# chonlei/neural-ode-ion-channels

Measured on AMD Instinct MI355X. Metric: trajectories/sec (sinewave protocol, 100k steps), higher is better.
Workload: dtype f64

## Files before the change

### include/ionode.h

```cpp
#ifndef IONODE_H
#define IONODE_H

#include <stddef.h>
#include <stdint.h>

#ifdef __cplusplus
extern "C" {
#endif

#define IONODE_ABI_VERSION 10

#define IONODE_MODEL_HH2 0
#define IONODE_MODEL_MARKOV6 1
#define IONODE_MODEL_NNF 2
#define IONODE_MODEL_NND 3

#define IONODE_STATUS_OK 0
#define IONODE_STATUS_DT_UNDERFLOW 1
#define IONODE_STATUS_NONFINITE 2
#define IONODE_STATUS_MAX_STEPS 3

#define IONODE_OK 0
#define IONODE_ERR_ARG (-1)
#define IONODE_ERR_UNSUPPORTED (-2)
// ... 27 lines not shown
  double *ckpt;
  int32_t ckpt_cap;
  int32_t t_eval_exact;
  const double *sse_ref;
  double *sse_out;
  double max_step;
  const double *v_at_outputs;
  int64_t mlp_image_stride;
  int32_t traj_per_image;
  const int32_t *launch_order;
} ionode_desc;

#define IONODE_DEFAULT_MAX_TOTAL_STEPS 1000000

size_t ionode_mlp_packed_floats(int32_t mlp_layers, int32_t mlp_width);

int ionode_mlp_pack(const float *state_dict_flat, int32_t mlp_layers, int32_t mlp_width, float *packed);

int ionode_dopri5(const ionode_desc *d, const float *mlp_packed, const double *params, const double *prot_v,
                  const double *prot_t, const int32_t *prot_of_traj, const void *y0, const double *t_eval,
                  void *y_out, double *i_out, int32_t *status, int64_t *stats, void *stream);

int ionode_dense_defer_plan(const ionode_desc *d, int32_t want_current, int64_t out[2]);
int ionode_dopri5_deferred(const ionode_desc *d, const float *mlp_packed, const double *params, const double *prot_v,
                           const double *prot_t, const int32_t *prot_of_traj, const void *y0, const double *t_eval,
                           void *y_out, double *i_out, int32_t *status, int64_t *stats, void *stream, void *workspace,
                           int64_t workspace_bytes);

int ionode_protocol_at_outputs(const ionode_desc *d, const double *prot_v, const double *prot_t, const double *t_eval,
                               double *v_out, void *stream);

int ionode_launch_geometry(const ionode_desc *d, int32_t out[4]);

const char *ionode_kernel_name(const ionode_desc *d);

const char *ionode_last_kernel_name(void);

int32_t ionode_lane_wise_from(int32_t model, int32_t mlp_width);

const char *ionode_last_error(void);
int32_t ionode_abi_version(void);


size_t ionode_grad_image_floats(int32_t mlp_layers, int32_t mlp_width);
int ionode_grad_pack(const float *state_dict_flat, int32_t mlp_layers, int32_t mlp_width, float *image);

// ... 64 lines not shown
```

### neural-ode-ion-channels_amd/capi.py

```python
import ctypes as C
import os
import subprocess

import numpy as np
import torch

_HERE = os.path.dirname(os.path.abspath(__file__))
LIB_PATH = os.environ.get("IONODE_LIB") or os.path.join(_HERE, "libionode.so")

MODEL_HH2, MODEL_MARKOV6, MODEL_NNF, MODEL_NND = 0, 1, 2, 3
STATUS_OK, STATUS_DT_UNDERFLOW, STATUS_NONFINITE, STATUS_MAX_STEPS = 0, 1, 2, 3
STATUS_TEXT = {
    0: "ok",
    1: "underflow in dt",
    2: "non-finite values in state `y`",
    3: "max_num_steps exceeded",
}
ABI_VERSION = 10

EXPORTS = (
    "ionode_abi_version", "ionode_last_error", "ionode_mlp_packed_floats", "ionode_mlp_pack",
    "ionode_launch_geometry", "ionode_kernel_name", "ionode_last_kernel_name", "ionode_lane_wise_from", "ionode_dopri5", "ionode_protocol_at_outputs",
    "ionode_grad_image_floats", "ionode_grad_pack", "ionode_grad_record_floats", "ionode_dopri5_backward", "ionode_dopri5_backward_sse",
    "ionode_grad_packet_doubles", "ionode_dopri5_backward_recompute", "ionode_dopri5_backward_sweep",
    "ionode_dopri5_backward_sse_gc", "ionode_dopri5_backward_recompute_sse", "ionode_dopri5_backward_sweep_sse",
    "ionode_grad_partial_floats", "ionode_grad_reduce", "ionode_grad_reduce_unit", "ionode_grad_reduce_slabs", "ionode_grad_last_error",
    "ionode_regress_step", "ionode_adam_step", "ionode_image_refresh", "ionode_regress_plan",
    "ionode_dense_defer_plan", "ionode_dopri5_deferred",
)

SWEEP_BUFFERS = {
    "ionode_dopri5_backward": ("grad_image", "params", "prot_v", "prot_t", "prot_of_traj", "t_eval", "n_accepted", "grad_y", "state",
                               "records", "grad_params", "grad_y0"),
    "ionode_dopri5_backward_sse": ("params", "prot_v", "prot_t", "prot_of_traj", "t_eval", "n_accepted", "grad_sse", "state",
                                   "grad_params", "grad_y0"),
    "ionode_dopri5_backward_recompute": ("grad_image", "params", "prot_v", "prot_t", "prot_of_traj", "t_eval", "n_accepted", "grad_y",
                                         "records", "packets"),
    "ionode_dopri5_backward_sweep": ("grad_image", "params", "prot_v", "prot_t", "prot_of_traj", "t_eval", "n_accepted", "grad_y", "state",
                                     "records", "packets", "grad_params", "grad_y0"),
    "ionode_dopri5_backward_sse_gc": ("prot_v", "prot_t", "prot_of_traj", "t_eval", "n_accepted", "grad_sse", "packets", "sse_grad_y0"),
    "ionode_dopri5_backward_recompute_sse": ("grad_image", "params", "prot_v", "prot_t", "prot_of_traj", "t_eval", "n_accepted", "records",
                                             "packets"),
    "ionode_dopri5_backward_sweep_sse": ("grad_image", "params", "prot_v", "prot_t", "prot_of_traj", "t_eval", "n_accepted", "sse_grad_y0",
                                         "state", "records", "packets", "grad_params", "grad_y0"),
}


def n_state(model):
    return 6 if model == MODEL_MARKOV6 else 2


# ... 39 lines not shown
def lib():
    global _lib
    if _lib is None:
        if not os.path.exists(LIB_PATH):
            raise IonodeError(f"{LIB_PATH} is missing: run `python -c 'import __graft_entry__ as g; g.build()'` "
                              "(there is no CPU fallback for the integrator)")
        L = C.CDLL(LIB_PATH)
        L.ionode_abi_version.restype = C.c_int32
        L.ionode_last_error.restype = C.c_char_p
        L.ionode_kernel_name.restype = C.c_char_p
        L.ionode_kernel_name.argtypes = [C.POINTER(IonodeDesc)]
        L.ionode_mlp_packed_floats.restype = C.c_size_t
        L.ionode_mlp_packed_floats.argtypes = [C.c_int32, C.c_int32]
        L.ionode_mlp_pack.restype = C.c_int
        L.ionode_mlp_pack.argtypes = [C.c_void_p, C.c_int32, C.c_int32, C.c_void_p]
        L.ionode_launch_geometry.restype = C.c_int
        L.ionode_launch_geometry.argtypes = [C.POINTER(IonodeDesc), C.POINTER(C.c_int32 * 4)]
        L.ionode_dopri5.restype = C.c_int
        L.ionode_dopri5.argtypes = [C.POINTER(IonodeDesc)] + [C.c_void_p] * 12
        L.ionode_dopri5_deferred.restype = C.c_int
        L.ionode_dopri5_deferred.argtypes = [C.POINTER(IonodeDesc)] + [C.c_void_p] * 13 + [C.c_int64]
        L.ionode_dense_defer_plan.restype = C.c_int
        L.ionode_dense_defer_plan.argtypes = [C.POINTER(IonodeDesc), C.c_int32, C.POINTER(C.c_int64 * 2)]
        L.ionode_grad_last_error.restype = C.c_char_p
        for fn in (L.ionode_grad_image_floats, L.ionode_grad_record_floats, L.ionode_grad_partial_floats):
            fn.restype = C.c_size_t
            fn.argtypes = [C.c_int32, C.c_int32]
        L.ionode_grad_pack.restype = C.c_int
        L.ionode_grad_pack.argtypes = [C.c_void_p, C.c_int32, C.c_int32, C.c_void_p]
        L.ionode_grad_packet_doubles.restype = C.c_size_t
        L.ionode_grad_packet_doubles.argtypes = []
        for name, buffers in SWEEP_BUFFERS.items():
            getattr(L, name).restype = C.c_int
            getattr(L, name).argtypes = [C.POINTER(IonodeDesc), C.c_int32, C.c_int32, C.c_int32] + [C.c_void_p] * (len(buffers) + 1)
        L.ionode_grad_reduce.restype = C.c_int
        L.ionode_grad_reduce.argtypes = [C.c_int32, C.c_int32, C.c_void_p, C.c_int64, C.c_int32, C.c_void_p, C.c_void_p]
        L.ionode_grad_reduce_slabs.restype = C.c_int32
        L.ionode_grad_reduce_slabs.argtypes = [C.c_int32, C.c_int32, C.c_int64]
        L.ionode_grad_reduce_unit.restype = C.c_int
        L.ionode_grad_reduce_unit.argtypes = [C.c_int32, C.c_int32, C.c_void_p, C.c_int64, C.c_int32, C.c_void_p, C.c_void_p]
        L.ionode_regress_step.restype = C.c_int
        L.ionode_regress_step.argtypes = [C.c_int32, C.c_int32, C.c_void_p, C.c_void_p, C.c_void_p, C.c_void_p, C.c_int32,
                                          C.c_float, C.c_void_p, C.c_void_p, C.c_int32, C.c_void_p]
        L.ionode_regress_plan.restype = C.c_int
        L.ionode_regress_plan.argtypes = [C.c_int32, C.c_int32, C.POINTER(C.c_int32 * 3)]
        L.ionode_adam_step.restype = C.c_int
# ... 49 lines not shown

def launch_geometry(desc):
    out = (C.c_int32 * 4)()
    rc = lib().ionode_launch_geometry(C.byref(desc), C.byref(out))
    if rc != 0:
        raise IonodeError(last_error())
    return {"grid": out[0], "block": out[1], "lds_bytes": out[2], "tile_waves": out[3]}


def regress_plan(mlp_layers, mlp_width):
    out = (C.c_int32 * 3)()
    if lib().ionode_regress_plan(int(mlp_layers), int(mlp_width), C.byref(out)) != 0:
        raise IonodeError(lib().ionode_grad_last_error().decode())
    return {"generic": bool(out[0]), "wg_per_cu": out[1], "lds_bytes": out[2]}


def dense_defer_plan(desc, want_current):
    out = (C.c_int64 * 2)()
    if lib().ionode_dense_defer_plan(C.byref(desc), int(bool(want_current)), C.byref(out)) != 0:
        raise IonodeError(last_error())
    return {"capacity": int(out[0]), "workspace_bytes": int(out[1])}


def kernel_name(desc):
    return lib().ionode_kernel_name(C.byref(desc)).decode()


def _dev_ptr(t, dtype, name, shape=None):
    if t is None:
        return None
    if not isinstance(t, torch.Tensor) or not t.is_cuda:
        raise IonodeError(f"{name}: expected a CUDA/HIP tensor (the integrator has no CPU path)")
    if t.dtype != dtype or not t.is_contiguous():
        raise IonodeError(f"{name}: expected contiguous {dtype}, got {t.dtype} contiguous={t.is_contiguous()}")
    if shape is not None and tuple(t.shape) != tuple(shape):
        raise IonodeError(f"{name}: expected shape {tuple(shape)}, got {tuple(t.shape)}")
    return C.c_void_p(t.data_ptr())


_order_cache = {}


def _protocol_major(prot_of_traj):
    key = (prot_of_traj.data_ptr(), prot_of_traj._version, int(prot_of_traj.shape[0]), str(prot_of_traj.device))
    hit = _order_cache.get(key)
    if hit is None:
        p = prot_of_traj.to(torch.int64)
        if bool((p[1:] >= p[:-1]).all()):
            hit = (None,)
        else:
            order = torch.argsort(p, stable=True)
            n = int(order.shape[0])
            if n % (64 * 8) == 0:
                order = order.view(8, n // (64 * 8), 64).transpose(0, 1).reshape(-1)
            hit = (order.to(torch.int32).contiguous(),)
        if len(_order_cache) > 8:
            _order_cache.clear()
        _order_cache[key] = hit
    return hit[0]


def dopri5(model, params, prot_v, y0, t_eval, *, mlp_packed=None, mlp_layers=0, mlp_width=0, prot_t=None,
           prot_t0=0.0, prot_dt=1.0, prot_of_traj=None, rtol=1e-7, atol=1e-9, v_oob=-80.0, max_steps=0,
           max_total_steps=0, max_step=0.0, ckpt=None, current=False, obs_g=1.0, obs_e=-86.0, obs_open_state_only=False, tile_waves=0, stats=True,
           step_log=None, t_eval_hint="auto", t_eval_exact=None, sse_ref=None, states=True, out=None, stream=None,
           v_at_outputs="auto", traj_per_image=0, launch_order="auto"):
    if not torch.cuda.is_available():
        raise IonodeError("no HIP device visible: ionode has no CPU fallback")
    B, D = y0.shape
    Nt = t_eval.shape[0]
    P, Np = prot_v.shape
    sdt = y0.dtype
    if sdt not in (torch.float32, torch.float64):
        raise IonodeError("y0 must be float32 or float64")
    desc = make_desc(model=model, state_f32=int(sdt == torch.float32), n_state=D, n_out=Nt, n_traj=B, n_prot=P,
                     prot_n=Np, mlp_layers=mlp_layers, mlp_width=mlp_width, n_params=params.shape[1],
                     max_steps=max_steps, max_total_steps=max_total_steps, max_step=max_step, prot_t0=prot_t0, prot_dt=prot_dt, v_oob=v_oob, rtol=rtol, atol=atol,
                     obs_g=obs_g, obs_e=obs_e, obs_open_state_only=int(obs_open_state_only), tile_waves=tile_waves)
    if traj_per_image:
        if mlp_packed is None or mlp_packed.dim() != 2 or mlp_packed.shape[0] * traj_per_image < B or not mlp_packed.is_contiguous():
            raise IonodeError("traj_per_image needs a contiguous mlp_packed [n_images, floats] with n_images * traj_per_image >= B")
        desc.mlp_image_stride, desc.traj_per_image = int(mlp_packed.shape[1]), int(traj_per_image)
    if isinstance(t_eval_hint, str) and t_eval_hint == "auto":
        t_eval_hint = uniform_grid(t_eval)
        if t_eval_hint is not None and t_eval_exact is None:
            t_eval_exact = t_eval_hint[2] == 0.0
    if t_eval_hint is not None and t_eval_hint[1] > 0:
        desc.t_eval_t0_hint, desc.t_eval_dt_hint = float(t_eval_hint[0]), float(t_eval_hint[1])
        if t_eval_exact is None:
# ... 37 lines not shown
    if current and i_out is None:
        i_out = torch.empty((B, Nt), dtype=torch.float64, device=dev)
    status = out.get("status")
    if status is None:
        status = torch.empty((B,), dtype=torch.int32, device=dev)
    st = out.get("stats")
    if stats and st is None:
        st = torch.empty((B, 4), dtype=torch.int64, device=dev)
    s = stream if stream is not None else torch.cuda.current_stream(dev).cuda_stream
    vtab = None
    if (current or sse_ref is not None) and model in (MODEL_HH2, MODEL_MARKOV6) and v_at_outputs is not None:
        if isinstance(v_at_outputs, str):
            if 4 * P <= B:
                vtab = protocol_at_outputs(desc, prot_v, prot_t, t_eval, stream=s)
        else:
            vtab = v_at_outputs
            _dev_ptr(vtab, torch.float64, "v_at_outputs", (P, Nt))
        if vtab is not None:
            desc.v_at_outputs = vtab.data_ptr()
    ws = None
    if stream is None and prot_t is None and y is not None:
        plan = dense_defer_plan(desc, i_out is not None)
        if plan["capacity"] > 0:
            ws = torch.empty((plan["workspace_bytes"],), dtype=torch.uint8, device=dev)
    rc = lib().ionode_dopri5_deferred(
        C.byref(desc),
        _dev_ptr(mlp_packed, torch.float32, "mlp_packed"),
        _dev_ptr(params, torch.float64, "params", (B, params.shape[1])),
        _dev_ptr(prot_v, torch.float64, "prot_v"),
        _dev_ptr(prot_t, torch.float64, "prot_t", (Np,)) if prot_t is not None else None,
        _dev_ptr(prot_of_traj, torch.int32, "prot_of_traj", (B,)) if prot_of_traj is not None else None,
        _dev_ptr(y0, sdt, "y0"),
        _dev_ptr(t_eval, torch.float64, "t_eval"),
        _dev_ptr(y, sdt, "y_out", (B, Nt, D)) if y is not None else None,
        _dev_ptr(i_out, torch.float64, "i_out", (B, Nt)) if i_out is not None else None,
        _dev_ptr(status, torch.int32, "status", (B,)),
        _dev_ptr(st, torch.int64, "stats", (B, 4)) if st is not None else None,
        C.c_void_p(s),
        C.c_void_p(ws.data_ptr()) if ws is not None else None,
        ws.numel() if ws is not None else 0,
    )
    if rc != 0:
        raise IonodeError(f"ionode_dopri5 failed ({rc}): {last_error()}")
    return {"y": y, "i": i_out, "status": status, "stats": st, "sse": sse, "desc": desc, "v_at_outputs": vtab,
            "kernel": lib().ionode_last_kernel_name().decode()}


# ... 31 lines not shown
```

### neural-ode-ion-channels_amd/csrc/ionode_attempt_body.hpp

```cpp
#ifdef IONODE_STAMPS
    constexpr int NET = std::is_same<typename std::decay<decltype(IONODE_NET)>::type, MlpShrink4>::value ? 1 : 0;
    const unsigned long long att0_ = stamp_now();
#endif
    if constexpr (LW) {
#pragma unroll
      for (int i = 0; i < NPAR; ++i) asm volatile("" : "+v"(p[i]));
    }
    bool failed_now = false;
    if (active) {
      if ((int64_t)since >= a.max_steps || (int64_t)nacc + nrej >= a.max_total) { status = IONODE_STATUS_MAX_STEPS; failed_now = true; }
      else if (!(t + dt > t)) { status = IONODE_STATUS_DT_UNDERFLOW; failed_now = true; }
      else {
        bool fin = true;
#pragma unroll
        for (int d = 0; d < D; ++d) fin = fin && isfinite((double)y[d]);
        if (!fin) { status = IONODE_STATUS_NONFINITE; failed_now = true; }
      }
      if (failed_now) active = false;
    }
    {
      unsigned long long fm = __ballot(failed_now && lane < LPS);
      while (fm) {
        const int jj = __builtin_ctzll(fm);
        fm &= fm - 1;
// ... 144 lines not shown
      int n_out = 0;
      if (acc_now) {
        const double gf = floor((t1 - a.te_t0) * a.te_rdt);
        long long g = (gf < (double)(oi - 1)) ? (long long)(oi - 1) : ((gf > (double)(Nt - 1)) ? (long long)(Nt - 1) : (long long)gf);
        if ((LW && LEAN && D > 2) || (!LW && a.te_exact)) {
          while (g >= oi && te_at((int)g) > t1) --g;
          while (g + 1 < Nt && te_at((int)g + 1) <= t1) ++g;
        } else {
          while (g >= oi && a.t_eval[g] > t1) --g;
          while (g + 1 < Nt && a.t_eval[g + 1] <= t1) ++g;
        }
        n_out = (int)(g - oi + 1);
      }
      STAMP(stamps_, 9);
      if constexpr (!LW && G > 1) {
      constexpr int NS = (LPS >= WPS) ? LPS / WPS : 1;
      const bool exact = a.te_exact != 0;
      const bool want_i = (a.i_out != nullptr) || (a.sse_out != nullptr);
      const bool ugrid = a.prot_t == nullptr;
      int n_emit = n_out;
      if constexpr (F::defer) {
        if (a.defer_rec != nullptr) {
          using Rec = DenseRecord<D>;
          const bool rec_now = n_out > 0 && nrec < a.defer_cap;
          const int rq = lane >> 4;
          auto chunk = [&](int r) {
            if (r == 0) return make_double2(t0, den);
            if (r == 1) return make_double2(rden, Rec::pack_cursor(oi_before, n_out));
            const int e = 2 * (r - 2);
            return make_double2((double)ic[e / D][e % D], (double)ic[(e + 1) / D][(e + 1) % D]);
          };
          double2 *__restrict__ row = reinterpret_cast<double2 *>(a.defer_rec + ((size_t)traj * (size_t)a.defer_cap + (size_t)nrec) * Rec::ROW);
#pragma unroll
          for (int w = 0; 4 * w < Rec::CHUNKS; ++w) {
            if (wis == w) {
              double2 v = chunk(4 * w);
#pragma unroll
              for (int qq = 1; qq < 4; ++qq) {
                if (4 * w + qq < Rec::CHUNKS) {
                  const double2 c = chunk(4 * w + qq);
                  if (rq == qq) v = c;
                }
              }
              if (rec_now && 4 * w + rq < Rec::CHUNKS) row[4 * w + rq] = v;
            }
          }
          if (rec_now) { n_emit = 0; ++nrec; }
// ... 412 lines not shown
```

### neural-ode-ion-channels_amd/csrc/ionode_capi.hip

```cpp
#include <algorithm>
#include <cstdio>
#include <cstdlib>
#include <cstring>
#include <vector>

#include "ionode_launch.hpp"

namespace {

constexpr int kTile32From = 8192;
constexpr int kTile4Upto = 1024;
constexpr int kTile1Upto = 256;
constexpr int kTiny64From = 32769;
constexpr int kHh2LaneFrom = 49152;
constexpr int kMarkov6LaneFrom = 24576;

thread_local char g_err[256] = "";
thread_local const char *g_last_kernel = "";

void set_err(const char *fmt, const char *detail = "") { snprintf(g_err, sizeof g_err, fmt, detail); }

inline int np_of(int N) { return 16 * ((N + 15) / 16); }

struct Plan {
// ... 132 lines not shown

struct DeferPlan {
  int64_t cap = 0, bytes = 0;
};
DeferPlan plan_defer(const ionode_desc *d, const Plan &pl, bool want_i) {
  DeferPlan p;
  if (!pl.v->defer || d->sse_out != nullptr || d->n_state != 2) return p;
  const char *sw = getenv("IONODE_DEFER_DENSE");
  if (sw != nullptr && sw[0] != '\0' && atoi(sw) == 0) return p;
  using Rec = ionode::DenseRecord<2>;
  const int64_t B = d->n_traj, Nt = d->n_out;
  const char *fc = getenv("IONODE_DEFER_DENSE_CAP");
  int64_t cap = (fc != nullptr && fc[0] != '\0') ? atoll(fc) : 0;
  const bool forced = cap > 0;
  if (!forced) {
    const int64_t out_bytes = B * Nt * 2 * (d->state_f32 ? 4 : 8) + (want_i ? B * Nt * 8 : 0);
    cap = (out_bytes / 4) / (B * Rec::BYTES);
  }
  cap = std::min<int64_t>(cap, Nt - 1);
  if (cap < (forced ? 1 : 64)) return p;
  p.cap = cap;
  p.bytes = (int64_t)Rec::workspace_bytes(B, cap);
  return p;
}

int make_plan(const ionode_desc *d, Plan *pl, bool want_current = false, bool explicit_grid = false) {
  if (!d) { set_err("null descriptor"); return IONODE_ERR_ARG; }
#ifdef IONODE_STAMPS
  const bool has_step_log = false;
#else
  const bool has_step_log = d->step_log != nullptr;
#endif
  const bool mlp = d->model == IONODE_MODEL_NNF || d->model == IONODE_MODEL_NND;
  const int D = d->model == IONODE_MODEL_MARKOV6 ? 6 : 2;
  if (d->model < 0 || d->model > 3) { set_err("unknown model"); return IONODE_ERR_ARG; }
  if (d->n_state != D) { set_err("n_state does not match model"); return IONODE_ERR_ARG; }
  if (d->n_traj < 1 || d->n_out < 1 || d->n_prot < 1 || d->prot_n < 2) { set_err("empty batch / grid / protocol"); return IONODE_ERR_ARG; }
  if (d->n_params < (D == 6 ? 12 : 8)) { set_err("n_params too small for model"); return IONODE_ERR_ARG; }
  if (!(d->rtol > 0) || !(d->atol >= 0) || !(d->prot_dt > 0)) { set_err("rtol/atol/prot_dt must be positive"); return IONODE_ERR_ARG; }
  const Ask k = {want_current, explicit_grid, has_step_log};
  return mlp ? plan_mlp(d, pl, k) : plan_closed(d, pl, k, D);
}

}

namespace ionode {
// ... 235 lines not shown
  return IONODE_OK;
}

const char *ionode_kernel_name(const ionode_desc *d) {
  Plan pl;
  if (make_plan(d, &pl, d && (d->sse_out != nullptr || d->v_at_outputs != nullptr)) != IONODE_OK) return "";
  return pl.v->name;
}

const char *ionode_last_kernel_name(void) { return g_last_kernel; }

int32_t ionode_lane_wise_from(int32_t model, int32_t mlp_width) { return lane_wise_from(model, mlp_width); }

int ionode_dense_defer_plan(const ionode_desc *d, int32_t want_current, int64_t out[2]) {
  Plan pl;
  const int rc = make_plan(d, &pl, want_current != 0 || (d && d->sse_out != nullptr));
  if (rc != IONODE_OK) return rc;
  const DeferPlan dp = plan_defer(d, pl, want_current != 0);
  out[0] = dp.cap;
  out[1] = dp.bytes;
  return IONODE_OK;
}

}

namespace {

int dopri5_impl(const ionode_desc *d, const float *mlp_packed, const double *params, const double *prot_v,
                const double *prot_t, const int32_t *prot_of_traj, const void *y0, const double *t_eval,
                void *y_out, double *i_out, int32_t *status, int64_t *stats, void *stream, void *workspace, int64_t workspace_bytes) {
  Plan pl;
  const int rc = make_plan(d, &pl, i_out != nullptr || d->sse_out != nullptr, prot_t != nullptr);
  if (rc != IONODE_OK) return rc;
  const bool mlp = d->model == IONODE_MODEL_NNF || d->model == IONODE_MODEL_NND;
  if (!params || !prot_v || !y0 || !t_eval || (!y_out && !d->sse_out) || !status || (mlp && !mlp_packed)) {
    set_err("ionode_dopri5: required buffer is NULL");
    return IONODE_ERR_ARG;
  }
  if (d->sse_out && (!d->sse_ref || !(d->t_eval_dt_hint > 0.0) || d->n_out < 2)) {
    set_err("fused objective: sse_out needs sse_ref and the output-grid hint (t_eval_dt_hint > 0)");
    return IONODE_ERR_ARG;
  }
  ionode::KArgs a;
  memset(&a, 0, sizeof a);
  a.mlp = mlp_packed; a.params = params; a.prot_v = prot_v; a.prot_t = prot_t; a.prot_of_traj = prot_of_traj;
  a.y0 = y0; a.t_eval = t_eval; a.y_out = y_out; a.i_out = i_out; a.status = status; a.stats = stats;
// ... 10 lines not shown
  a.obs_g = d->obs_g; a.obs_e = d->obs_e; a.obs_open = d->obs_open_state_only;
  a.step_log = d->step_log; a.step_log_cap = d->step_log ? d->step_log_cap : 0;
  a.sse_ref = d->sse_ref; a.sse_out = d->sse_out; a.v_tab = d->v_at_outputs;
  if (mlp && d->traj_per_image > 0) { a.mlp_stride = d->mlp_image_stride; a.traj_per_img = d->traj_per_image; }
  if (d->launch_order) {
    if (a.traj_per_img > 0) { set_err("launch_order cannot be combined with traj_per_image (tiles of an image must stay together)"); return IONODE_ERR_ARG; }
    a.order = d->launch_order;
  }
  a.lw_bytes = (int32_t)pl.lw_bytes;
  a.te_t0 = d->t_eval_t0_hint; a.te_dt = (d->t_eval_dt_hint > 0.0 && d->n_out > 1) ? d->t_eval_dt_hint : 0.0;
  a.te_rdt = a.te_dt > 0.0 ? 1.0 / a.te_dt : 0.0;
  a.te_exact = (a.te_dt > 0.0 && d->t_eval_exact) ? 1 : 0;
  a.tile_shrink = pl.tile_shrink ? 1 : 0;
  DeferPlan dp;
  if (workspace != nullptr && prot_t == nullptr && y_out != nullptr) dp = plan_defer(d, pl, i_out != nullptr);
  if (dp.cap > 0) {
    if (workspace_bytes < dp.bytes || (reinterpret_cast<uintptr_t>(workspace) & 15) != 0) {
      set_err("ionode_dopri5_deferred: workspace smaller than ionode_dense_defer_plan() asks for, or not 16-byte aligned");
      return IONODE_ERR_ARG;
    }
    a.defer_count = static_cast<int32_t *>(workspace);
    a.defer_rec = reinterpret_cast<double *>(static_cast<unsigned char *>(workspace) + ionode::DenseRecord<2>::records_offset(d->n_traj));
    a.defer_cap = (int32_t)dp.cap;
  }
  hipError_t e = pl.v->fn(a, pl.grid, pl.lds, reinterpret_cast<hipStream_t>(stream));
  if (e != hipSuccess) { set_err("kernel launch failed: %s", hipGetErrorString(e)); return IONODE_ERR_LAUNCH; }
  if (dp.cap > 0) {
    const dim3 grid((unsigned)std::min<int64_t>((dp.cap + ionode::kExpandRecordsPerWg - 1) / ionode::kExpandRecordsPerWg, ionode::kExpandMaxBlocks),
                    (unsigned)std::min(d->n_traj, 65535));
    if (d->state_f32) hipLaunchKernelGGL((ionode::ionode_dense_expand_kernel<float, 2>), grid, dim3(256), 0, reinterpret_cast<hipStream_t>(stream), a);
    else hipLaunchKernelGGL((ionode::ionode_dense_expand_kernel<double, 2>), grid, dim3(256), 0, reinterpret_cast<hipStream_t>(stream), a);
    e = hipGetLastError();
    if (e != hipSuccess) { set_err("kernel launch failed: %s", hipGetErrorString(e)); return IONODE_ERR_LAUNCH; }
  }
  g_last_kernel = pl.v->name;
  return IONODE_OK;
}

}

extern "C" {

int ionode_dopri5(const ionode_desc *d, const float *mlp_packed, const double *params, const double *prot_v,
                  const double *prot_t, const int32_t *prot_of_traj, const void *y0, const double *t_eval,
                  void *y_out, double *i_out, int32_t *status, int64_t *stats, void *stream) {
  return dopri5_impl(d, mlp_packed, params, prot_v, prot_t, prot_of_traj, y0, t_eval, y_out, i_out, status, stats, stream, nullptr, 0);
}

int ionode_dopri5_deferred(const ionode_desc *d, const float *mlp_packed, const double *params, const double *prot_v,
                           const double *prot_t, const int32_t *prot_of_traj, const void *y0, const double *t_eval,
                           void *y_out, double *i_out, int32_t *status, int64_t *stats, void *stream, void *workspace,
                           int64_t workspace_bytes) {
// ... 22 lines not shown
```

### neural-ode-ion-channels_amd/csrc/ionode_dense_expand.hpp

```cpp
#pragma once

#include <hip/hip_runtime.h>
#include <stdint.h>

#include "ionode_kargs.hpp"
#include "ionode_math.hpp"

namespace ionode {

template <int D> struct DenseRecord {
  static constexpr int ROW = 4 + 5 * D;
  static constexpr int BYTES = ROW * 8;
  static constexpr int CHUNKS = ROW / 2;
  static constexpr int T0 = 0, DEN = 1, RDEN = 2, CURSOR = 3, COEF = 4;
  static_assert(ROW % 2 == 0, "records are whole 16-byte chunks");
  static __host__ __device__ constexpr size_t records_offset(int64_t B) { return ((size_t)B * 4 + 15) & ~(size_t)15; }
  static __host__ __device__ constexpr size_t workspace_bytes(int64_t B, int64_t cap) { return records_offset(B) + (size_t)B * (size_t)cap * BYTES; }
  static __device__ __forceinline__ double pack_cursor(int oi_before, int n_out) { return __hiloint2double(n_out, oi_before); }
  static __device__ __forceinline__ int cursor_oi(double w) { return __double2loint(w); }
  static __device__ __forceinline__ int cursor_n(double w) { return __double2hiint(w); }
};

constexpr int kExpandRecordsPerWg = 16;
constexpr int kExpandMaxBlocks = 128;

template <typename S, int D> __global__ void __launch_bounds__(256) ionode_dense_expand_kernel(const KArgs a) {
  using Rec = DenseRecord<D>;
  const int lane = threadIdx.x & 63;
  const int wv = __builtin_amdgcn_readfirstlane(threadIdx.x >> 6);
  const int Nt = a.Nt;
  auto te_at = [&](int idx) -> double { return a.te_t0 + (double)idx * a.te_dt; };
  const bool want_i = a.i_out != nullptr;
  for (int tr = (int)blockIdx.y; tr < a.B; tr += (int)gridDim.y) {
    int cnt = a.defer_count[tr];
    cnt = cnt < a.defer_cap ? cnt : a.defer_cap;
    if ((int)blockIdx.x * kExpandRecordsPerWg >= cnt) continue;
    const int pj = a.prot_of_traj ? a.prot_of_traj[tr] : (tr % a.P);
    const double *__restrict__ pv = a.prot_v + (size_t)pj * a.Np;
    S *__restrict__ yo = a.y_out ? reinterpret_cast<S *>(a.y_out) + (size_t)tr * Nt * D : nullptr;
    double *__restrict__ io = a.i_out ? a.i_out + (size_t)tr * Nt : nullptr;
    for (int r0 = (int)blockIdx.x * kExpandRecordsPerWg; r0 < cnt; r0 += (int)gridDim.x * kExpandRecordsPerWg) {
    const int r1 = (r0 + kExpandRecordsPerWg < cnt) ? r0 + kExpandRecordsPerWg : cnt;
    for (int ri = r0 + wv; ri < r1; ri += 4) {
      const double *__restrict__ rec = a.defer_rec + ((size_t)tr * (size_t)a.defer_cap + (size_t)ri) * Rec::ROW;
      const double t0b = rec[Rec::T0], denb = rec[Rec::DEN], rdenb = rec[Rec::RDEN];
      const double cur = rec[Rec::CURSOR];
      const int o = Rec::cursor_oi(cur), n = Rec::cursor_n(cur);
      S cb[5][D];
#pragma unroll
      for (int c = 0; c < 5; ++c)
#pragma unroll
        for (int d = 0; d < D; ++d) cb[c][d] = (S)rec[Rec::COEF + c * D + d];
      for (int c0 = 0; c0 < n; c0 += 64) {
        const int idx = o + c0 + lane;
        if (c0 + lane < n && idx < Nt) {
          const double tk = te_at(idx);
          const S x = (S)div_pos(tk - t0b, denb, rdenb);
          S out[D];
          S xp = x;
#pragma unroll
          for (int d = 0; d < D; ++d) out[d] = cb[0][d] + x * cb[1][d];
#pragma unroll
          for (int c = 2; c < 5; ++c) {
            xp = xp * x;
#pragma unroll
            for (int d = 0; d < D; ++d) out[d] = out[d] + xp * cb[c][d];
          }
          if (yo) {
            if constexpr (sizeof(S) == 8) {
#pragma unroll
              for (int d = 0; d < D; d += 2) *reinterpret_cast<double2 *>(yo + (size_t)idx * D + d) = make_double2(out[d], out[d + 1]);
            } else {
#pragma unroll
              for (int d = 0; d < D; d += 2) *reinterpret_cast<float2 *>(yo + (size_t)idx * D + d) = make_float2(out[d], out[d + 1]);
            }
          }
          if (want_i) {
            int ip;
            const bool inr = protocol_index(a, tk, ip);
            const double vk = inr ? protocol_from(a, pv[ip - 1], pv[ip], ip, tk) : a.v_oob;
            S gate;
            if (a.obs_open) gate = out[D - 1]; else gate = out[0] * out[1];
            if (a.obs_g != 1.0) gate = (S)a.obs_g * gate;
            io[idx] = (double)gate * (vk - a.obs_e);
          }
        }
      }
    }
    }
  }
}

}
```

### neural-ode-ion-channels_amd/csrc/ionode_device.hpp

```cpp
#pragma once

#include <hip/hip_runtime.h>
#include <stdint.h>

#include <type_traits>

#include "../../include/ionode.h"
#include "ionode_form.hpp"
#include "ionode_kargs.hpp"
#include "ionode_math.hpp"
#include "ionode_dense_expand.hpp"

namespace ionode {

struct LwLds {
  static __host__ __device__ constexpr int rowb(int D) { return (4 + 5 * D) * 8; }
  static __host__ __device__ constexpr int aux_off(int D) { return 64 * rowb(D); }
  static __host__ __device__ constexpr int aux_bytes(int tail) { return (tail == 1 && IONODE_LEAN) ? 0 : 64 * 64; }
  static __host__ __device__ constexpr int owp_off(int D, int tail) { return aux_off(D) + aux_bytes(tail); }
  static __host__ __device__ constexpr int trl_off(int D, int tail) { return owp_off(D, tail) + 256; }
  static __host__ __device__ constexpr int clist_off(int D, int tail) { return trl_off(D, tail) + 256; }
  static __host__ __device__ constexpr int bytes(int D, int tail) { return clist_off(D, tail) + 1024; }
};
static_assert(LwLds::rowb(2) == DenseRecord<2>::BYTES && LwLds::rowb(6) == DenseRecord<6>::BYTES, "the deferred-output record is the lane-wise kernels' row");
// ... 51 lines not shown
  const int wave = LW ? 0 : wgw;
  const int tile = LW ? (int)((blockIdx.x & 7u) + 8u * ((blockIdx.x >> 3) * (unsigned)IONODE_LW_TILES_PER_WG + (unsigned)wgw)) : (int)blockIdx.x;
  unsigned char *const smem_t = LW ? smem + (size_t)wgw * (size_t)a.lw_bytes : smem;
  if constexpr (LW) {
    if (tile * TPW >= a_in.B) return;
  }
  const int j = lane % LPS;
  const int cset = (NSETS > 1) ? wave / WPS : 0, wis = wave % WPS;
  const bool primary = (lane < LPS) && (wis == 0);
  const int slot_raw = tile * TPW + cset * LPS + j;
  const bool valid = slot_raw < a.B;
  const int slot_c = valid ? slot_raw : a.B - 1;
  const int traj = a.order ? a.order[slot_c] : slot_c;
  const int traj_raw = valid ? traj : a.B;

  using MlpT = typename F::Mlp;
  MlpT mlp;
  if constexpr (MT::MLP) mlp.init(a, smem_t, wave, lane, tile * TPW);
  size_t lw_off = 0;
  if constexpr (T64) lw_off = (MlpT::lds_bytes(a.L) + 15) & ~(size_t)15;
  unsigned char *const lsm = smem_t + lw_off;
  STAMP_DECL
#ifdef IONODE_STAMPS
  if constexpr (MT::MLP) mlp.sp = &stamps_;
#endif

  double p[NPAR];
#pragma unroll
  for (int i = 0; i < NPAR; ++i) p[i] = a.params[(size_t)traj * a.n_params + i];
  const int pidx = a.prot_of_traj ? a.prot_of_traj[traj] : (traj % a.P);
  const double *__restrict__ pv = a.prot_v + (size_t)pidx * a.Np;

  const S rtol = (S)a.rtol, atol = (S)a.atol;
  S *__restrict__ yout = reinterpret_cast<S *>(a.y_out) + (size_t)traj * a.Nt * D;
  double *__restrict__ iout = a.i_out ? a.i_out + (size_t)traj * a.Nt : nullptr;
  const int Nt = a.Nt;

  S y[D], f[D];
#pragma unroll
  for (int d = 0; d < D; ++d) y[d] = reinterpret_cast<const S *>(a.y0)[(size_t)traj * D + d];

  double t = a.t_eval[0];
  {
    double v0;
    const bool in0 = protocol_v(a, pv, (double)(S)t, v0);
    rhs<MODEL, S, T64>(a, p, v0, in0, y, f, mlp);
// ... 155 lines not shown
  if (threadIdx.x == 0 && a.step_log != nullptr) {
    if (blockIdx.x == 0 && a.step_log_cap >= 9) {
      a.step_log[32] = (double)att_cyc[0]; a.step_log[33] = (double)att_n[0];
      a.step_log[34] = (double)att_cyc[1]; a.step_log[35] = (double)att_n[1];
    }
    if (4 * a.step_log_cap >= 64 + (int64_t)gridDim.x) a.step_log[64 + blockIdx.x] = (double)att_n[1];
  }
#ifdef IONODE_ASM_STAMPS
  if constexpr (MT::MLP && G == 4 && NT == 13) {
    unsigned sv_;
    asm volatile("v_accvgpr_read_b32 %0, a92" : "=v"(sv_));
    if (blockIdx.x == 0 && threadIdx.x < 16 && a.step_log != nullptr && a.step_log_cap >= 8) a.step_log[16 + threadIdx.x] = (double)sv_;
  }
#endif
#endif
  if constexpr (LW) {
    if (a.sse_out != nullptr) {
#pragma unroll
      for (int m = 0; m < 8; ++m) sse += ssep[j * 8 + m];
    }
  }
  if (a.sse_out != nullptr && valid && lane < LPS && (WPS == 1 || (lane % WPS) == wis))
    a.sse_out[traj] = (status == IONODE_STATUS_OK) ? sse : __builtin_inf();
  if constexpr (F::defer) {
    if (a.defer_rec != nullptr && valid && primary) a.defer_count[traj] = nrec;
  }
  if (valid && primary) {
    a.status[traj] = status;
    if (a.stats) {
      int64_t *st = a.stats + (size_t)traj * 4;
      st[0] = nacc;
      st[1] = nrej;
      st[2] = 2 + 6 * ((int64_t)nacc + nrej);
      st[3] = status;
    }
  }
}

}
```

### neural-ode-ion-channels_amd/csrc/ionode_kargs.hpp

```cpp
#pragma once

#include <hip/hip_runtime.h>
#include <stdint.h>

#include "../../include/ionode.h"
#include "ionode_form.hpp"
#include "ionode_math.hpp"

namespace ionode {

struct KArgs {
  const float *mlp;
  const double *params;
  const double *prot_v;
  const double *prot_t;
  const int32_t *prot_of_traj;
  const void *y0;
  const double *t_eval;
  void *y_out;
  double *i_out;
  int32_t *status;
  int64_t *stats;
  int32_t B, Nt, P, Np, n_params, L, N, NP, NT;
  int64_t max_steps;
  int64_t max_total;
  double *ckpt;
  int32_t ckpt_cap;
  double prot_t0, prot_dt, v_oob, rtol, atol, obs_g, obs_e;
  double prot_rdt;
  double dt_max;
  int32_t obs_open;
  double *step_log;
  int64_t step_log_cap;
  const double *sse_ref;
  double *sse_out;
  double te_t0, te_dt;
  double te_rdt;
  int32_t te_exact;
  const double *v_tab;
  int64_t mlp_stride;
  int32_t traj_per_img;
  int32_t lw_bytes;
  const int32_t *order;
  int32_t tile_shrink;
  int32_t *defer_count;
  double *defer_rec;
  int32_t defer_cap;
};

__device__ __forceinline__ bool protocol_index(const KArgs &a, double t, int &i);
__device__ __forceinline__ double protocol_from(const KArgs &a, double v_lo, double v_hi, int i, double t);

__device__ __forceinline__ bool protocol_index(const KArgs &a, double t, int &i) {
  const int n = a.Np;
  const double t_last = a.prot_t0 + (double)(n - 1) * a.prot_dt;
  const bool inr = !(t < a.prot_t0 || t > t_last || t != t);
  const double u = div_by(t - a.prot_t0, a.prot_dt, a.prot_rdt);
  double ci = ceil(u);
  ci = (ci < 1.0) ? 1.0 : ci;
  ci = (ci > (double)(n - 1)) ? (double)(n - 1) : ci;
  i = inr ? (int)ci : 1;
  return inr;
}
__device__ __forceinline__ double protocol_from(const KArgs &a, double v_lo, double v_hi, int i, double t) {
  const double x_lo = a.prot_t0 + (double)(i - 1) * a.prot_dt;
  const double slope = div_by(v_hi - v_lo, a.prot_dt, a.prot_rdt);
  return slope * (t - x_lo) + v_lo;
}

__device__ __forceinline__ bool protocol_v(const KArgs &a, const double *__restrict__ pv, double t, double &v) {
// ... 22 lines not shown
```

Before: 12590.

## Expand deferred dense output in-kernel for early-finishing tiles, flatten expand grid

```diff
diff --git a/include/ionode.h b/include/ionode.h
--- a/include/ionode.h
+++ b/include/ionode.h
@@ -73,6 +73,7 @@
                   void *y_out, double *i_out, int32_t *status, int64_t *stats, void *stream);
 
 int ionode_dense_defer_plan(const ionode_desc *d, int32_t want_current, int64_t out[2]);
+int ionode_dense_tail_plan(const ionode_desc *d, int32_t want_current, int64_t out[2]);
 int ionode_dopri5_deferred(const ionode_desc *d, const float *mlp_packed, const double *params, const double *prot_v,
                            const double *prot_t, const int32_t *prot_of_traj, const void *y0, const double *t_eval,
                            void *y_out, double *i_out, int32_t *status, int64_t *stats, void *stream, void *workspace,
diff --git a/neural-ode-ion-channels_amd/capi.py b/neural-ode-ion-channels_amd/capi.py
--- a/neural-ode-ion-channels_amd/capi.py
+++ b/neural-ode-ion-channels_amd/capi.py
@@ -26,7 +26,7 @@
     "ionode_dopri5_backward_sse_gc", "ionode_dopri5_backward_recompute_sse", "ionode_dopri5_backward_sweep_sse",
     "ionode_grad_partial_floats", "ionode_grad_reduce", "ionode_grad_reduce_unit", "ionode_grad_reduce_slabs", "ionode_grad_last_error",
     "ionode_regress_step", "ionode_adam_step", "ionode_image_refresh", "ionode_regress_plan",
-    "ionode_dense_defer_plan", "ionode_dopri5_deferred",
+    "ionode_dense_defer_plan", "ionode_dense_tail_plan", "ionode_dopri5_deferred",
 )
 
 SWEEP_BUFFERS = {
@@ -112,6 +112,8 @@
         L.ionode_dopri5_deferred.argtypes = [C.POINTER(IonodeDesc)] + [C.c_void_p] * 13 + [C.c_int64]
         L.ionode_dense_defer_plan.restype = C.c_int
         L.ionode_dense_defer_plan.argtypes = [C.POINTER(IonodeDesc), C.c_int32, C.POINTER(C.c_int64 * 2)]
+        L.ionode_dense_tail_plan.restype = C.c_int
+        L.ionode_dense_tail_plan.argtypes = [C.POINTER(IonodeDesc), C.c_int32, C.POINTER(C.c_int64 * 2)]
         L.ionode_grad_last_error.restype = C.c_char_p
         for fn in (L.ionode_grad_image_floats, L.ionode_grad_record_floats, L.ionode_grad_partial_floats):
             fn.restype = C.c_size_t
@@ -207,6 +209,13 @@
     return {"capacity": int(out[0]), "workspace_bytes": int(out[1])}
 
 
+def dense_tail_plan(desc, want_current):
+    out = (C.c_int64 * 2)()
+    if lib().ionode_dense_tail_plan(C.byref(desc), int(bool(want_current)), C.byref(out)) != 0:
+        raise IonodeError(last_error())
+    return {"tail_rank": int(out[0]), "usable_capacity": int(out[1])}
+
+
 def kernel_name(desc):
     return lib().ionode_kernel_name(C.byref(desc)).decode()
 
@@ -249,7 +258,7 @@
            prot_t0=0.0, prot_dt=1.0, prot_of_traj=None, rtol=1e-7, atol=1e-9, v_oob=-80.0, max_steps=0,
            max_total_steps=0, max_step=0.0, ckpt=None, current=False, obs_g=1.0, obs_e=-86.0, obs_open_state_only=False, tile_waves=0, stats=True,
            step_log=None, t_eval_hint="auto", t_eval_exact=None, sse_ref=None, states=True, out=None, stream=None,
-           v_at_outputs="auto", traj_per_image=0, launch_order="auto"):
+           v_at_outputs="auto", traj_per_image=0, launch_order="auto", workspace=None):
     if not torch.cuda.is_available():
         raise IonodeError("no HIP device visible: ionode has no CPU fallback")
     B, D = y0.shape
@@ -333,7 +342,11 @@
     if stream is None and prot_t is None and y is not None:
         plan = dense_defer_plan(desc, i_out is not None)
         if plan["capacity"] > 0:
-            ws = torch.empty((plan["workspace_bytes"],), dtype=torch.uint8, device=dev)
+            if workspace is not None:
+                _dev_ptr(workspace, torch.uint8, "workspace")
+                if workspace.numel() < plan["workspace_bytes"]:
+                    raise IonodeError(f"workspace: {workspace.numel()} bytes, the plan asks for {plan['workspace_bytes']}")
+            ws = workspace if workspace is not None else torch.empty((plan["workspace_bytes"],), dtype=torch.uint8, device=dev)
     rc = lib().ionode_dopri5_deferred(
         C.byref(desc),
         _dev_ptr(mlp_packed, torch.float32, "mlp_packed"),
diff --git a/neural-ode-ion-channels_amd/csrc/ionode_attempt_body.hpp b/neural-ode-ion-channels_amd/csrc/ionode_attempt_body.hpp
--- a/neural-ode-ion-channels_amd/csrc/ionode_attempt_body.hpp
+++ b/neural-ode-ion-channels_amd/csrc/ionode_attempt_body.hpp
@@ -190,7 +190,7 @@
       if constexpr (F::defer) {
         if (a.defer_rec != nullptr) {
           using Rec = DenseRecord<D>;
-          const bool rec_now = n_out > 0 && nrec < a.defer_cap;
+          const bool rec_now = n_out > 0 && nrec < a.defer_fill;
           const int rq = lane >> 4;
           auto chunk = [&](int r) {
             if (r == 0) return make_double2(t0, den);
diff --git a/neural-ode-ion-channels_amd/csrc/ionode_capi.hip b/neural-ode-ion-channels_amd/csrc/ionode_capi.hip
--- a/neural-ode-ion-channels_amd/csrc/ionode_capi.hip
+++ b/neural-ode-ion-channels_amd/csrc/ionode_capi.hip
@@ -178,6 +178,27 @@
   p.cap = cap;
   p.bytes = (int64_t)Rec::workspace_bytes(B, cap);
   return p;
+}
+
+constexpr int64_t kDeferTailEighths = 5;
+struct TailPlan {
+  int64_t rank = 0, fill = 0;
+};
+TailPlan plan_tail(const Plan &pl, const DeferPlan &dp) {
+  TailPlan t;
+  t.fill = dp.cap;
+  if (dp.cap < 2) return t;
+  const int64_t tiles = (int64_t)pl.grid;
+  t.rank = tiles * kDeferTailEighths / 8;
+  const char *fr = getenv("IONODE_DEFER_TAIL_RANK");
+  if (fr != nullptr && fr[0] != '\0') t.rank = std::max<int64_t>(0, std::min<int64_t>(atoll(fr), tiles));
+  const char *sw = getenv("IONODE_DEFER_TAIL");
+  if (sw != nullptr && sw[0] != '\0') {
+    if (strcmp(sw, "all") == 0) t.rank = tiles;
+    else if (atoi(sw) == 0) t.rank = 0;
+  }
+  if (t.rank > 0) t.fill = dp.cap - 1;
+  return t;
 }
 
 int make_plan(const ionode_desc *d, Plan *pl, bool want_current = false, bool explicit_grid = false) {
@@ -459,6 +480,16 @@
   return IONODE_OK;
 }
 
+int ionode_dense_tail_plan(const ionode_desc *d, int32_t want_current, int64_t out[2]) {
+  Plan pl;
+  const int rc = make_plan(d, &pl, want_current != 0 || (d && d->sse_out != nullptr));
+  if (rc != IONODE_OK) return rc;
+  const TailPlan tp = plan_tail(pl, plan_defer(d, pl, want_current != 0));
+  out[0] = tp.rank;
+  out[1] = tp.fill;
+  return IONODE_OK;
+}
+
 }
 
 namespace {
@@ -515,12 +546,20 @@
     a.defer_count = static_cast<int32_t *>(workspace);
     a.defer_rec = reinterpret_cast<double *>(static_cast<unsigned char *>(workspace) + ionode::DenseRecord<2>::records_offset(d->n_traj));
     a.defer_cap = (int32_t)dp.cap;
+    const TailPlan tp = plan_tail(pl, dp);
+    a.defer_fill = (int32_t)tp.fill;
+    a.defer_tail_rank = (int32_t)tp.rank;
+    if (tp.rank > 0) {
+      a.defer_tail = reinterpret_cast<int32_t *>(a.defer_rec + ((size_t)d->n_traj * (size_t)dp.cap - 1) * ionode::DenseRecord<2>::ROW);
+      const hipError_t em = hipMemsetAsync(a.defer_tail, 0, ionode::DenseRecord<2>::BYTES, reinterpret_cast<hipStream_t>(stream));
+      if (em != hipSuccess) { set_err("hipMemsetAsync failed: %s", hipGetErrorString(em)); return IONODE_ERR_LAUNCH; }
+    }
   }
   hipError_t e = pl.v->fn(a, pl.grid, pl.lds, reinterpret_cast<hipStream_t>(stream));
   if (e != hipSuccess) { set_err("kernel launch failed: %s", hipGetErrorString(e)); return IONODE_ERR_LAUNCH; }
   if (dp.cap > 0) {
-    const dim3 grid((unsigned)std::min<int64_t>((dp.cap + ionode::kExpandRecordsPerWg - 1) / ionode::kExpandRecordsPerWg, ionode::kExpandMaxBlocks),
-                    (unsigned)std::min(d->n_traj, 65535));
+    const int64_t blocks = std::min<int64_t>((dp.cap + ionode::kExpandRecordsPerWg - 1) / ionode::kExpandRecordsPerWg, ionode::kExpandMaxBlocks);
+    const dim3 grid((unsigned)std::min<int64_t>((int64_t)d->n_traj * blocks, ionode::kExpandGrid));
     if (d->state_f32) hipLaunchKernelGGL((ionode::ionode_dense_expand_kernel<float, 2>), grid, dim3(256), 0, reinterpret_cast<hipStream_t>(stream), a);
     else hipLaunchKernelGGL((ionode::ionode_dense_expand_kernel<double, 2>), grid, dim3(256), 0, reinterpret_cast<hipStream_t>(stream), a);
     e = hipGetLastError();
diff --git a/neural-ode-ion-channels_amd/csrc/ionode_dense_expand.hpp b/neural-ode-ion-channels_amd/csrc/ionode_dense_expand.hpp
--- a/neural-ode-ion-channels_amd/csrc/ionode_dense_expand.hpp
+++ b/neural-ode-ion-channels_amd/csrc/ionode_dense_expand.hpp
@@ -21,72 +21,128 @@
   static __device__ __forceinline__ int cursor_n(double w) { return __double2hiint(w); }
 };
 
-constexpr int kExpandRecordsPerWg = 16;
+#ifndef IONODE_EXPAND_RECORDS_PER_WG
+#define IONODE_EXPAND_RECORDS_PER_WG 64
+#endif
+constexpr int kExpandRecordsPerWg = IONODE_EXPAND_RECORDS_PER_WG;
 constexpr int kExpandMaxBlocks = 128;
+constexpr int kExpandGrid = 256 * 8;
+constexpr int kExpandAheadKernel = 4;
+constexpr int kExpandAheadTail = 8;
+
+template <typename S, int D, int K>
+__device__ __forceinline__ void dense_expand_records(const KArgs &a, int tr, int r0, int r1, int step, int lane) {
+  using Rec = DenseRecord<D>;
+  static_assert(Rec::ROW <= 64, "one lane per double of a record");
+  if (r0 >= r1) return;
+  const int Nt = a.Nt;
+  const bool want_i = a.i_out != nullptr;
+  const int pj = a.prot_of_traj ? a.prot_of_traj[tr] : (tr % a.P);
+  const double *__restrict__ pv = a.prot_v + (size_t)pj * a.Np;
+  S *__restrict__ yo = a.y_out ? reinterpret_cast<S *>(a.y_out) + (size_t)tr * Nt * D : nullptr;
+  double *__restrict__ io = a.i_out ? a.i_out + (size_t)tr * Nt : nullptr;
+  const double *__restrict__ recs = a.defer_rec + (size_t)tr * (size_t)a.defer_cap * Rec::ROW + (lane < Rec::ROW ? lane : Rec::ROW - 1);
+  const int last = r0 + ((r1 - 1 - r0) / step) * step;
+  auto fetch = [&](int ri) -> double { return recs[(size_t)(ri < last ? ri : last) * Rec::ROW]; };
+  struct Head {
+    double t0, den, rden;
+    int o, n;
+    S cb[5][D];
+  };
+  struct Samples {
+    double tk, lo, hi;
+    int ip;
+    bool inr;
+  };
+  auto decode = [&](double raw, Head &h) {
+    h.t0 = bcast_f64(raw, Rec::T0); h.den = bcast_f64(raw, Rec::DEN); h.rden = bcast_f64(raw, Rec::RDEN);
+    const double cur = bcast_f64(raw, Rec::CURSOR);
+    h.o = Rec::cursor_oi(cur); h.n = Rec::cursor_n(cur);
+#pragma unroll
+    for (int c = 0; c < 5; ++c)
+#pragma unroll
+      for (int d = 0; d < D; ++d) h.cb[c][d] = (S)bcast_f64(raw, Rec::COEF + c * D + d);
+  };
+  auto lookup = [&](const Head &h, int c0, Samples &s) {
+    s.tk = a.te_t0 + (double)(h.o + c0 + lane) * a.te_dt;
+    s.lo = s.hi = 0.0; s.ip = 1; s.inr = false;
+    if (want_i) {
+      s.inr = protocol_index(a, s.tk, s.ip);
+      s.lo = pv[s.ip - 1]; s.hi = pv[s.ip];
+    }
+  };
+  auto emit = [&](const Head &h, int c0, const Samples &s) {
+    const int idx = h.o + c0 + lane;
+    if (c0 + lane < h.n && idx < Nt) {
+      const double tk = s.tk;
+      const S x = (S)div_pos(tk - h.t0, h.den, h.rden);
+      S out[D];
+      S xp = x;
+#pragma unroll
+      for (int d = 0; d < D; ++d) out[d] = h.cb[0][d] + x * h.cb[1][d];
+#pragma unroll
+      for (int c = 2; c < 5; ++c) {
+        xp = xp * x;
+#pragma unroll
+        for (int d = 0; d < D; ++d) out[d] = out[d] + xp * h.cb[c][d];
+      }
+      if (yo) {
+        if constexpr (sizeof(S) == 8) {
+#pragma unroll
+          for (int d = 0; d < D; d += 2) *reinterpret_cast<double2 *>(yo + (size_t)idx * D + d) = make_double2(out[d], out[d + 1]);
+        } else {
+#pragma unroll
+          for (int d = 0; d < D; d += 2) *reinterpret_cast<float2 *>(yo + (size_t)idx * D + d) = make_float2(out[d], out[d + 1]);
+        }
+      }
+      if (want_i) {
+        const double vk = s.inr ? protocol_from(a, s.lo, s.hi, s.ip, tk) : a.v_oob;
+        S gate;
+        if (a.obs_open) gate = out[D - 1]; else gate = out[0] * out[1];
+        if (a.obs_g != 1.0) gate = (S)a.obs_g * gate;
+        io[idx] = (double)gate * (vk - a.obs_e);
+      }
+    }
+  };
+  double raw[K];
+#pragma unroll
+  for (int k = 0; k < K; ++k) raw[k] = fetch(r0 + k * step);
+  Head hc, hn;
+  Samples sc, sn;
+  decode(raw[0], hc);
+  lookup(hc, 0, sc);
+  for (int ri = r0; ri < r1; ri += K * step) {
+#pragma unroll
+    for (int k = 0; k < K; ++k) {
+      const int rk = ri + k * step;
+      if (rk >= r1) break;
+      raw[k] = fetch(rk + K * step);
+      decode(raw[(k + 1) % K], hn);
+      lookup(hn, 0, sn);
+      emit(hc, 0, sc);
+      for (int c0 = 64; c0 < hc.n; c0 += 64) {
+        Samples s;
+        lookup(hc, c0, s);
+        emit(hc, c0, s);
+      }
+      hc = hn; sc = sn;
+    }
+  }
+}
 
 template <typename S, int D> __global__ void __launch_bounds__(256) ionode_dense_expand_kernel(const KArgs a) {
-  using Rec = DenseRecord<D>;
   const int lane = threadIdx.x & 63;
   const int wv = __builtin_amdgcn_readfirstlane(threadIdx.x >> 6);
-  const int Nt = a.Nt;
-  auto te_at = [&](int idx) -> double { return a.te_t0 + (double)idx * a.te_dt; };
-  const bool want_i = a.i_out != nullptr;
-  for (int tr = (int)blockIdx.y; tr < a.B; tr += (int)gridDim.y) {
+  const int nblk = (a.defer_cap + kExpandRecordsPerWg - 1) / kExpandRecordsPerWg;
+  const int bpt = nblk < kExpandMaxBlocks ? nblk : kExpandMaxBlocks;
+  const long long pairs = (long long)a.B * bpt;
+  for (long long pr = blockIdx.x; pr < pairs; pr += gridDim.x) {
+    const int tr = (int)(pr / bpt), b0 = (int)(pr % bpt);
     int cnt = a.defer_count[tr];
     cnt = cnt < a.defer_cap ? cnt : a.defer_cap;
-    if ((int)blockIdx.x * kExpandRecordsPerWg >= cnt) continue;
-    const int pj = a.prot_of_traj ? a.prot_of_traj[tr] : (tr % a.P);
-    const double *__restrict__ pv = a.prot_v + (size_t)pj * a.Np;
-    S *__restrict__ yo = a.y_out ? reinterpret_cast<S *>(a.y_out) + (size_t)tr * Nt * D : nullptr;
-    double *__restrict__ io = a.i_out ? a.i_out + (size_t)tr * Nt : nullptr;
-    for (int r0 = (int)blockIdx.x * kExpandRecordsPerWg; r0 < cnt; r0 += (int)gridDim.x * kExpandRecordsPerWg) {
-    const int r1 = (r0 + kExpandRecordsPerWg < cnt) ? r0 + kExpandRecordsPerWg : cnt;
-    for (int ri = r0 + wv; ri < r1; ri += 4) {
-      const double *__restrict__ rec = a.defer_rec + ((size_t)tr * (size_t)a.defer_cap + (size_t)ri) * Rec::ROW;
-      const double t0b = rec[Rec::T0], denb = rec[Rec::DEN], rdenb = rec[Rec::RDEN];
-      const double cur = rec[Rec::CURSOR];
-      const int o = Rec::cursor_oi(cur), n = Rec::cursor_n(cur);
-      S cb[5][D];
-#pragma unroll
-      for (int c = 0; c < 5; ++c)
-#pragma unroll
-        for (int d = 0; d < D; ++d) cb[c][d] = (S)rec[Rec::COEF + c * D + d];
-      for (int c0 = 0; c0 < n; c0 += 64) {
-        const int idx = o + c0 + lane;
-        if (c0 + lane < n && idx < Nt) {
-          const double tk = te_at(idx);
-          const S x = (S)div_pos(tk - t0b, denb, rdenb);
-          S out[D];
-          S xp = x;
-#pragma unroll
-          for (int d = 0; d < D; ++d) out[d] = cb[0][d] + x * cb[1][d];
-#pragma unroll
-          for (int c = 2; c < 5; ++c) {
-            xp = xp * x;
-#pragma unroll
-            for (int d = 0; d < D; ++d) out[d] = out[d] + xp * cb[c][d];
-          }
-          if (yo) {
-            if constexpr (sizeof(S) == 8) {
-#pragma unroll
-              for (int d = 0; d < D; d += 2) *reinterpret_cast<double2 *>(yo + (size_t)idx * D + d) = make_double2(out[d], out[d + 1]);
-            } else {
-#pragma unroll
-              for (int d = 0; d < D; d += 2) *reinterpret_cast<float2 *>(yo + (size_t)idx * D + d) = make_float2(out[d], out[d + 1]);
-            }
-          }
-          if (want_i) {
-            int ip;
-            const bool inr = protocol_index(a, tk, ip);
-            const double vk = inr ? protocol_from(a, pv[ip - 1], pv[ip], ip, tk) : a.v_oob;
-            S gate;
-            if (a.obs_open) gate = out[D - 1]; else gate = out[0] * out[1];
-            if (a.obs_g != 1.0) gate = (S)a.obs_g * gate;
-            io[idx] = (double)gate * (vk - a.obs_e);
-          }
-        }
-      }
-    }
+    for (int r0 = b0 * kExpandRecordsPerWg; r0 < cnt; r0 += bpt * kExpandRecordsPerWg) {
+      const int r1 = (r0 + kExpandRecordsPerWg < cnt) ? r0 + kExpandRecordsPerWg : cnt;
+      dense_expand_records<S, D, kExpandAheadKernel>(a, tr, r0 + wv, r1, 4, lane);
     }
   }
 }
diff --git a/neural-ode-ion-channels_amd/csrc/ionode_device.hpp b/neural-ode-ion-channels_amd/csrc/ionode_device.hpp
--- a/neural-ode-ion-channels_amd/csrc/ionode_device.hpp
+++ b/neural-ode-ion-channels_amd/csrc/ionode_device.hpp
@@ -97,6 +97,7 @@
   unsigned char *const lsm = smem_t + lw_off;
   STAMP_DECL
 #ifdef IONODE_STAMPS
+  [[maybe_unused]] const unsigned long long wall0_ = wall_clock64();
   if constexpr (MT::MLP) mlp.sp = &stamps_;
 #endif
 
@@ -298,9 +299,6 @@
   }
   if (a.sse_out != nullptr && valid && lane < LPS && (WPS == 1 || (lane % WPS) == wis))
     a.sse_out[traj] = (status == IONODE_STATUS_OK) ? sse : __builtin_inf();
-  if constexpr (F::defer) {
-    if (a.defer_rec != nullptr && valid && primary) a.defer_count[traj] = nrec;
-  }
   if (valid && primary) {
     a.status[traj] = status;
     if (a.stats) {
@@ -311,6 +309,41 @@
       st[3] = status;
     }
   }
+  if constexpr (F::defer) {
+    if (a.defer_rec != nullptr) {
+      int left = nrec;
+      if (a.defer_tail_rank > 0) {
+        asm volatile("s_waitcnt vmcnt(0) lgkmcnt(0)" ::: "memory");
+        __syncthreads();
+        int *const rank_lds = reinterpret_cast<int *>(smem);
+        if (threadIdx.x == 0) *rank_lds = atomicAdd(a.defer_tail, 1);
+        __syncthreads();
+        const int rank = __builtin_amdgcn_readfirstlane(*rank_lds);
+#ifdef IONODE_STAMPS
+        const unsigned long long wall1_ = wall_clock64();
+#endif
+        if (rank < a.defer_tail_rank) {
+          __threadfence();
+          __syncthreads();
+          __threadfence();
+#pragma unroll 1
+          for (int jj = 0; jj < LPS; ++jj) {
+            const int cj = __builtin_amdgcn_readlane(nrec, jj);
+            if (cj > 0) dense_expand_records<S, D, kExpandAheadTail>(a, __builtin_amdgcn_readlane(traj, jj), wave, cj, G, lane);
+          }
+          left = -(nrec + 1);
+        }
+#ifdef IONODE_STAMPS
+        if (threadIdx.x == 0 && a.step_log != nullptr && 4 * a.step_log_cap >= 64 + 4 * (int64_t)gridDim.x) {
+          double *const w_ = a.step_log + 64 + gridDim.x + 3 * (size_t)blockIdx.x;
+          asm volatile("s_waitcnt vmcnt(0)" ::: "memory");
+          w_[0] = (double)wall0_; w_[1] = (double)wall1_; w_[2] = (double)wall_clock64();
+        }
+#endif
+      }
+      if (valid && primary) a.defer_count[traj] = left;
+    }
+  }
 }
 
 }
diff --git a/neural-ode-ion-channels_amd/csrc/ionode_kargs.hpp b/neural-ode-ion-channels_amd/csrc/ionode_kargs.hpp
--- a/neural-ode-ion-channels_amd/csrc/ionode_kargs.hpp
+++ b/neural-ode-ion-channels_amd/csrc/ionode_kargs.hpp
@@ -46,6 +46,9 @@
   int32_t *defer_count;
   double *defer_rec;
   int32_t defer_cap;
+  int32_t defer_fill;
+  int32_t defer_tail_rank;
+  int32_t *defer_tail;
 };
 
 __device__ __forceinline__ bool protocol_index(const KArgs &a, double t, int &i);
```

New measurement: 12750, median of 6. 1.3% higher.
